# uga-ssrl/SSRLCV

Measured on AMD Instinct MI355X. Metric: Mpix/s SIFT extract (+ Mmatches/s 128-D brute-force, see `matcher`), higher is better.
Workload: dtype f32; 1 GPU; 2-view 4096x4096 pair per GPU (tools/scene.py pinhole views (PCG32 terrain + texture through Image::Camera)): SIFT_FeatureFactory::generateFeatures (sparse DoG path) on each image, pixels resident in HBM; images_per_gpu=2, parallelism=image-pair shard, library=release build (libssrlcv_hip_release.so)

## Files before the change

ssrlcv_amd/csrc/keypoints.hip:

```cpp
#include <hip/hip_runtime.h>
#include <float.h>
#include <math.h>
#include <stdlib.h>
#include "compact.h"
#include "dev_switch.h"
#include "scan_lookback.h"
#include "device_math.h"
#include "sift_plan.h"
#include "ssrlcv_hip.h"

using svp::OctaveState;

namespace {

struct LevelSet {
  const float* lvl[svp::kGauss];
  const float* lvlMinMax;
  const float* minmax;
  const float2* polar;
  int w, h;
};

struct DogView {
  const float* lo;
// ... 470 lines not shown
      tab->start[r] = pos;
      pos += count;
    }
  }
  tab->total = pos;
}
__device__ __forceinline__ int range_of(const RangeTable* tab, uint32_t u) {
  int r = 0;
#pragma unroll
  for (int k = 1; k < 20; ++k)
    if (tab->start[k] <= u) r = k;
  return r;
}

struct OctaveSet {
  LevelSet L[svp::kOctaves];
  const ssrlcv_sskeypoint* kps[svp::kOctaves];
  float pixelWidth[svp::kOctaves];
  float* thetas[svp::kOctaves];
  uint32_t* thetaCnt[svp::kOctaves];
  const void* consts[svp::kOctaves];
};

template <int MAXO, int LPKS>
__global__ __launch_bounds__(64) void k_thetas(const OctaveState* states, const RangeTable* tab, OctaveSet set, float lambda,
                                               float orientationThreshold) {
  constexpr int LANES = 1 << LPKS, PER_BLOCK = 64 >> LPKS, CW = kThetaChunk * LANES;
  __shared__ float s_hist[36][PER_BLOCK];
  if (blockIdx.x >= tab->total) return;
  const int range = __builtin_amdgcn_readfirstlane(range_of(tab, blockIdx.x));
  const int octave = range & 3, useg = kSegOrder[range >> 2];
  const LevelSet& L = set.L[octave];
  const float pixelWidth = set.pixelWidth[octave];
  const int t = threadIdx.x, sub = t & (LANES - 1), col = t >> LPKS;
  const float fsub2 = (float)(2 * sub);
  const uint32_t local = (blockIdx.x - tab->start[range]) * PER_BLOCK + (uint32_t)(t >> LPKS);
  const bool have = local < tab->count[range];
  const int gi = (int)(tab->first[range] + local);
  const float pi = SSRLCV_PI_F;
  const float rad10 = pi / 18.0f;
  const float inv10 = 1.0f / rad10;
  ssrlcv_sskeypoint kp;
  kp.loc.x = kp.loc.y = 0.0f;
  kp.sigma = 1.0f;
  if (have) kp = set.kps[octave][gi];
  const float kx = kp.loc.x, ky = kp.loc.y;
  const float windowWidth = ceilf(kp.sigma * 3.0f * lambda / pixelWidth);
  const float minx = kx - windowWidth, miny = ky - windowWidth, maxx = kx + windowWidth, maxy = ky + windowWidth;
  const bool inside = have && useg >= 1 && useg <= 3 &&
                      !(minx < 0.0f || miny < 0.0f || maxx >= (unsigned)(L.w - 1) || maxy >= (unsigned)(L.h - 1));
#pragma unroll
  for (int i = 0; i < 36 * PER_BLOCK / 64; ++i) (&s_hist[0][0])[i * 64 + t] = 0.0f;
  const float weight = 2.0f * lambda * lambda * kp.sigma * kp.sigma;
  const float rweight = 1.0f / weight;
  const int W = L.w;
  const size_t levelStride = svp::polar_level_stride(L.w, L.h);
  {
    const float2* base = L.polar + (size_t)(useg - 1) * levelStride;
    const __amdgpu_buffer_rsrc_t rsrc = __builtin_amdgcn_make_buffer_rsrc((void*)base, 0, (int)(uint32_t)(levelStride * 8), 0x00020000);
    typedef unsigned u32x4 __attribute__((ext_vector_type(4)));
    typedef unsigned u32x2 __attribute__((ext_vector_type(2)));
    struct Cursor { float x, y, ty2; unsigned rowoff; bool act; };
    Cursor cf;
    cf.x = minx;
    cf.y = miny;
    cf.ty2 = (miny - ky) * (miny - ky);
    cf.rowoff = (unsigned)round_pos(miny) * (unsigned)W + 1u;
    cf.act = inside;
    auto advance = [&](Cursor& c) {
      float xn = c.x + (float)CW;
      if (__any(c.act && !(c.x >= (float)CW))) {
        float ch = c.x;
#pragma unroll 8
        for (int i = 0; i < CW; ++i) ch += 1.0f;
        xn = c.x >= (float)CW ? xn : ch;
      }
      if (c.act) {
        if (xn <= maxx) {
          c.x = xn;
        } else {
          c.x = minx;
          c.y += 1.0f;
          if (!(c.y <= maxy)) c.act = false;
          const float ty = c.y - ky;
          c.ty2 = ty * ty;
          c.rowoff = (unsigned)round_pos(c.y) * (unsigned)W + 1u;
        }
      }
    };
    typedef u32x4 Chunk[kThetaChunk / 2];
    auto fetch = [&](const Cursor& c, Chunk& into) {
      if (!c.act) return;
      const unsigned off = (c.rowoff + (unsigned)round_pos(c.x)) * 8u + 16u * (unsigned)sub;
#pragma unroll
      for (int j = 0; j < kThetaChunk / 4; ++j) into[j] = __builtin_amdgcn_raw_buffer_load_b128(rsrc, (int)(off + 16u * LANES * j), 0, 0);
    };
    auto fetch_upper = [&](const Cursor& c, Chunk& into) {
      if (!c.act) return;
      const unsigned off = (c.rowoff + (unsigned)round_pos(c.x)) * 8u + 16u * (unsigned)sub;
#pragma unroll
      for (int j = kThetaChunk / 4; j < kThetaChunk / 2; ++j) into[j] = __builtin_amdgcn_raw_buffer_load_b128(rsrc, (int)(off + 16u * LANES * j), 0, 0);
    };
    auto wants_upper = [&](const Cursor& c) { return __any(c.act && c.x + (float)(CW / 2 - 1) <= maxx); };
    Chunk qa, qb;
    Cursor ca, cb;
#pragma unroll
    for (int j = 0; j < kThetaChunk / 2; ++j) qa[j] = qb[j] = u32x4{0u, 0u, 0u, 0u};
    ca = cf;
    fetch(cf, qa);
    if (wants_upper(cf)) fetch_upper(cf, qa);
    advance(cf);
    cb = cf;
    auto step = [&](Chunk& cur, const Cursor& cc, Chunk& nxt, Cursor& cn) __attribute__((always_inline)) {
      cn = cf;
      fetch(cf, nxt);
      if (wants_upper(cf)) fetch_upper(cf, nxt);
      advance(cf);
      float xs[kThetaChunk];
      float xlast = cc.x + (float)(CW - 1);
#pragma unroll
      for (int i = 0; i < kThetaChunk; ++i) xs[i] = cc.x + (fsub2 + (float)(((i >> 1) << (1 + LPKS)) | (i & 1)));
      if (__any(cc.act && !(cc.x >= (float)CW))) {
        float ch = cc.x;
        float xc[kThetaChunk];
#pragma unroll
        for (int sIdx = 0; sIdx < CW; ++sIdx) {
          const int q = (sIdx >> 1) & (LANES - 1), i = ((sIdx >> (1 + LPKS)) << 1) | (sIdx & 1);
          if (LANES == 1 || q == 0) xc[i] = ch;
          else xc[i] = sub == q ? ch : xc[i];
          if (sIdx + 1 < CW) ch += 1.0f;
        }
        const bool direct = cc.x >= (float)CW;
#pragma unroll
        for (int i = 0; i < kThetaChunk; ++i) xs[i] = direct ? xs[i] : xc[i];
        xlast = direct ? xlast : ch;
      }
      const float cty2 = cc.ty2;
      const unsigned crow = cc.rowoff;
      const bool cact = cc.act;
      const bool aligned = cc.x >= 4.0f && round_pos(xlast) == round_pos(cc.x) + (CW - 1);
      if (__any(cact && !aligned)) {
        if (cact && !aligned) {
#pragma unroll
          for (int i = 0; i < kThetaChunk; ++i) {
            u32x2 e = u32x2{0u, 0u};
            if (xs[i] <= maxx) e = __builtin_amdgcn_raw_buffer_load_b64(rsrc, (int)((crow + (unsigned)round_pos(xs[i])) * 8u), 0, 0);
            cur[i >> 1][(i & 1) * 2] = e[0];
            cur[i >> 1][(i & 1) * 2 + 1] = e[1];
          }
        }
      }
      auto weigh = [&](float ang, float xi, float& wgt, int& bin) {
        const float angle = fmod_2pi_above(ang + (2.0f * pi), 2.0f * pi);
        bin = (int)floorf(sv::exact_div3(angle, rad10, inv10));
        const float tx = xi - kx;
        wgt = sv::expf_nonpos(sv::exact_div5(-((tx * tx) + cty2), weight, rweight));
      };
      const bool upperHalf = __any(cact && xs[kThetaChunk / 2] <= maxx);
      float wg[kThetaChunk], mg[kThetaChunk];
      float* slot[kThetaChunk];
      auto weigh_half = [&](auto hc) __attribute__((always_inline)) {
        constexpr int i0 = decltype(hc)::value * (kThetaChunk / 2);
#pragma unroll
        for (int i = i0; i < i0 + kThetaChunk / 2; ++i) {
          const unsigned um = cur[i >> 1][(i & 1) * 2], ua = cur[i >> 1][(i & 1) * 2 + 1];
          int bin;
          weigh(__builtin_bit_cast(float, ua), xs[i], wg[i], bin);
          const bool counts = cact && xs[i] <= maxx && (unsigned)bin < 36u;
          slot[i] = &s_hist[counts ? bin : 0][col];
          mg[i] = counts ? __builtin_bit_cast(float, um) : 0.0f;
        }
      };
      auto vote_half = [&](auto hc) __attribute__((always_inline)) {
        constexpr int j0 = decltype(hc)::value * (kThetaChunk / 4);
#pragma unroll
        for (int j = j0; j < j0 + kThetaChunk / 4; ++j) {
#pragma unroll
          for (int q = 0; q < LANES; ++q) {
            if (LANES == 1 || sub == q) {
              const float h0 = *slot[2 * j], h1 = *slot[2 * j + 1];
              const float n0 = fmaf(mg[2 * j], wg[2 * j], h0);
              const float n1 = fmaf(mg[2 * j + 1], wg[2 * j + 1], slot[2 * j + 1] == slot[2 * j] ? n0 : h1);
              *slot[2 * j] = n0;
              *slot[2 * j + 1] = n1;
            }
            if (LANES > 1) __builtin_amdgcn_wave_barrier();
          }
        }
      };
      weigh_half(std::integral_constant<int, 0>{});
      if (upperHalf) weigh_half(std::integral_constant<int, 1>{});
      vote_half(std::integral_constant<int, 0>{});
      if (upperHalf) vote_half(std::integral_constant<int, 1>{});
    };
    while (__any(ca.act)) {
      step(qa, ca, qb, cb);
      if (!__any(cb.act)) break;
      step(qb, cb, qa, ca);
    }
  }
  uint32_t cnt = 0;
  float outTheta[MAXO];
#pragma unroll
  for (int i = 0; i < MAXO; ++i) outTheta[i] = -FLT_MAX;
  if (inside && sub == 0) {
    float maxHist = 0.0f;
    for (int i = 0; i < 36; ++i) {
      const float h = s_hist[i][col];
      if (h > maxHist) maxHist = h;
    }
    maxHist *= orientationThreshold;
    float bestMag[MAXO], bestTh[MAXO];
#pragma unroll
    for (int i = 0; i < MAXO; ++i) { bestMag[i] = 0.0f; bestTh[i] = 0.0f; }
    float hprev = s_hist[35][col], hb = s_hist[0][col];
    for (int b = 0; b < 36; ++b) {
      const float hnext = s_hist[b == 35 ? 0 : b + 1][col];
      if (!(hb < maxHist || hb < hprev || hb < hnext || hb < bestMag[MAXO - 1])) {
        float tmag = hb;
        float tt = (hprev - hnext) / (hprev - (2.0f * hb) + hnext);
        tt *= (pi / 36.0f);
        tt += (b * rad10);
        tt = fmodf(tt + (2.0f * pi), 2.0f * pi);
#pragma unroll
        for (int i = 0; i < MAXO; ++i) {
          if (tmag > bestMag[i]) {
#pragma unroll
            for (int ii = i; ii < MAXO; ++ii) {
              float m2 = bestMag[ii], t2 = bestTh[ii];
              bestMag[ii] = tmag;
              bestTh[ii] = tt;
              tmag = m2;
              tt = t2;
            }
          }
        }
      }
      hprev = hb;
      hb = hnext;
    }
#pragma unroll
    for (int i = 0; i < MAXO; ++i) {
      if (bestMag[i] != 0.0f) { outTheta[i] = bestTh[i]; cnt = i + 1; }
    }
  }
  if (have && sub == 0) {
#pragma unroll
    for (int i = 0; i < MAXO; ++i) set.thetas[octave][(size_t)gi * svp::kMaxOrient + i] = outTheta[i];
    set.thetaCnt[octave][gi] = cnt;
  }
}

__device__ __forceinline__ float uniform_f(float v) {
  return __builtin_bit_cast(float, __builtin_amdgcn_readfirstlane(__builtin_bit_cast(int, v)));
}
struct DescConst {
  float c, s;
  float windowWidth;
  float invExpDen;
  float voteScale;
  float invBin;
  uint32_t magic;
  int32_t segment;
};
static_assert(sizeof(DescConst) == 32, "one s_load_dwordx8");
__global__ __launch_bounds__(256) void k_desc_consts(const RangeTable* tab, OctaveSet set, float lambda, const OctaveState* states,
                                                     const GroupCtl* regularCtl) {
  const uint32_t total = tab->total;
  const bool fromTable = regularCtl != nullptr && regularCtl->regular != 0u;
  for (uint32_t u = blockIdx.x * 256 + threadIdx.x; u < total; u += gridDim.x * 256) {
    const int range = range_of(tab, u);
    const int octave = range & 3;
    const int i = (int)(tab->first[range] + (u - tab->start[range]));
    const ssrlcv_sskeypoint* kps = set.kps[octave];
    const float pixelWidth = set.pixelWidth[octave];
    DescConst* __restrict__ out = (DescConst*)const_cast<void*>(set.consts[octave]);
    DescConst d;
    const float theta = kps[i].theta;
    d.c = sv_cosf(-theta);
    d.s = sv_sinf(-theta);
    d.windowWidth = ceilf(kps[i].sigma * lambda / pixelWidth);
    d.invExpDen = 1.0f / (2.0f * d.windowWidth * d.windowWidth);
    int boundExp;
    (void)frexpf(1.4143f * ((d.windowWidth + 2.0f) * (d.windowWidth + 2.0f)), &boundExp);
    d.voteScale = ldexpf(1.0f, 31 - boundExp);
    d.invBin = 1.0f / (d.windowWidth / 2.0f);
    const unsigned wi = (unsigned)(int)d.windowWidth;
    d.magic = wi > 1u ? 0xFFFFFFFFu / wi + 1u : 0u;
    d.segment = fromTable ? kSegOrder[range >> 2] : segment_of(states + octave, i);
    out[i] = d;
  }
}

__device__ __forceinline__ unsigned vote_u32(float v) {
  int r;
  asm("v_cvt_rpi_i32_f32 %0, %1" : "=v"(r) : "v"(v));
  return (unsigned)r;
}

#ifndef SSRLCV_DESC_COPIES
#define SSRLCV_DESC_COPIES 8
#endif
constexpr int kDescCopies = SSRLCV_DESC_COPIES;
#ifndef SSRLCV_DESC_VGPRS
#define SSRLCV_DESC_VGPRS 64
#endif
__global__ __launch_bounds__(256) __attribute__((amdgpu_waves_per_eu(4, 8), amdgpu_num_vgpr(SSRLCV_DESC_VGPRS), amdgpu_num_sgpr(102))) void k_descriptors(const RangeTable* tab, OctaveSet set, const uint32_t* featBase,
                                                     ssrlcv_sift_feature* __restrict__ features, uint32_t maxFeatures) {
  __shared__ unsigned s_bins[4][(1 + 128 + 2) * kDescCopies];
  __shared__ __attribute__((aligned(8))) uint8_t s_bytes[4][128];
  const int lane = threadIdx.x & 63, wave = __builtin_amdgcn_readfirstlane(threadIdx.x >> 6);
  unsigned* bins = s_bins[wave] + kDescCopies;
  const int copy = lane & (kDescCopies - 1);
  const float pi = SSRLCV_PI_F;
  const float rad45 = pi / 4.0f;
  const float inv45 = 1.0f / rad45;
  const uint32_t totalUnits = tab->total;
  for (uint32_t unit = blockIdx.x * 4 + wave; unit < totalUnits; unit += gridDim.x * 4) {
    const int range = range_of(tab, unit);
    const int octave = range & 3;
    const int gi = (int)(tab->first[range] + (unit - tab->start[range]));
    const LevelSet& L = set.L[octave];
    const float pixelWidth = set.pixelWidth[octave];
    const float2* __restrict__ polar = L.polar;
    const DescConst dc = reinterpret_cast<const DescConst*>(set.consts[octave])[gi];
    const ssrlcv_sskeypoint kp = set.kps[octave][gi];
    const int seg = dc.segment;
    const float kx = kp.loc.x, ky = kp.loc.y;
    const float theta = kp.theta;
    const float windowWidth = dc.windowWidth;
    const float binWidth = windowWidth / 2.0f;
    const float c = dc.c, s = dc.s;
    const float2* __restrict__ pl = polar + (size_t)(seg - 1) * svp::polar_level_stride(L.w, L.h) + 1;
#pragma unroll
    for (int i = 0; i < 2 * kDescCopies; ++i) bins[i * 64 + lane] = 0u;
    f32x2 rc[16];
    {
      const int ci = lane & 15;
      const float hx = ((float)(ci >> 2) * 0.5f - 0.75f) * windowWidth, hy = ((float)(ci & 3) * 0.5f - 0.75f) * windowWidth;
      const float rx = (hx * c) + (hy * s), ry = (-hx * s) + (hy * c);
#pragma unroll
      for (int cell = 0; cell < 16; ++cell) {
        if ((cell >> 2) == 0 || (cell & 3) == 0) continue;
        rc[cell].x = __builtin_bit_cast(float, __builtin_amdgcn_readlane(__builtin_bit_cast(int, rx), cell));
        rc[cell].y = __builtin_bit_cast(float, __builtin_amdgcn_readlane(__builtin_bit_cast(int, ry), cell));
      }
    }
    const float expDen = 2.0f * windowWidth * windowWidth, invExpDen = dc.invExpDen, invBin = dc.invBin;
    const float voteScale = dc.voteScale;
    const int Wi = (int)windowWidth;
    const unsigned centreIdx = (unsigned)(Wi * (Wi + 1));
    const unsigned magic = dc.magic;
    auto sample = [&](unsigned idx, float& cx, float& cy, bool& ok) {
      const unsigned yq = Wi == 1 ? idx : __umulhi(idx, magic);
      const unsigned xq = idx - yq * (unsigned)Wi + 1u;
      const bool centre = idx >= centreIdx;
      const float x = centre ? 0.0f : (float)(int)xq;
      const float y = centre ? 0.0f : (float)(int)yq;
      cx = (x * c) + (y * s);
      cy = (-x * s) + (y * c);
      ok = idx <= centreIdx && fmaxf(fabsf(cx), fabsf(cy)) <= windowWidth;
    };
    auto gather = [&](float px, float py) { return polar_px(pl, L.w, round_coord(px), round_coord(py)); };
    auto split = [&](float2 pg, bool live, float& w0, float& w1, unsigned*& pa, float& ang, bool& odd) {
      ang = fmod_2pi_above(pg.y - theta + (2.0f * pi), 2.0f * pi);
      const float t45 = ang * inv45;
      const float fk = floorf(t45);
      const float u = t45 - fk;
      odd = live && !(u > 1.0e-4f && u < 0.9999f);
      int k0 = (int)fk;
      const float a0 = fabsf(ang - (fk * rad45)), a1 = fabsf(ang - ((fk + 1.0f) * rad45));
      w0 = (live && !odd && (unsigned)k0 < 8u) ? 1.0f - sv::exact_div3(a0, rad45, inv45) : 0.0f;
      w1 = (live && !odd && (unsigned)(k0 + 1) < 8u) ? 1.0f - sv::exact_div3(a1, rad45, inv45) : 0.0f;
      k0 = k0 < -1 ? -1 : k0;
      pa = bins + k0 * kDescCopies + copy;
    };
    float ncx, ncy;
    bool nok;
    sample((unsigned)lane, ncx, ncy, nok);
    float2 npg[4] = {make_float2(0.0f, 0.0f), make_float2(0.0f, 0.0f), make_float2(0.0f, 0.0f), make_float2(0.0f, 0.0f)};
    auto gather4 = [&]() {
      npg[0] = gather(ncx + kx, ncy + ky);
      npg[1] = gather(kx - ncy, ncx + ky);
      npg[2] = gather(kx - ncx, ky - ncy);
      npg[3] = gather(ncy + kx, ky - ncx);
    };
    if (nok) gather4();
    for (unsigned base = 0; base <= centreIdx; base += 64) {
      const float cx = ncx, cy = ncy;
      const bool ok = nok;
      const float2 pg0 = npg[0], pg1 = npg[1], pg2 = npg[2], pg3 = npg[3];
      const bool turned = ok && base + (unsigned)lane < centreIdx;
      sample(base + 64 + (unsigned)lane, ncx, ncy, nok);
      if (nok) gather4();
      const float r2n = -((cx * cx) + (cy * cy));
      const float g = sv::expf_nonpos(sv::exact_div3(r2n, expDen, invExpDen)) * voteScale;
      float a0, a1, b0, b1, c0, c1, d0, d1, angA, angB, angC, angD;
      bool oddA, oddB, oddC, oddD;
      unsigned *pa, *pb, *pc, *pd;
      split(pg0, ok, a0, a1, pa, angA, oddA);
      split(pg1, turned, b0, b1, pb, angB, oddB);
      split(pg2, turned, c0, c1, pc, angC, oddC);
      split(pg3, turned, d0, d1, pd, angD, oddD);
      const float magA = pg0.x * g, magB = pg1.x * g, magC = pg2.x * g, magD = pg3.x * g;
      const float bwl = ok ? binWidth : -1.0f;
#pragma unroll
      for (int cell = 0; cell < 16; ++cell) {
        const int nx = cell >> 2, ny = cell & 3;
        if (nx == 0 || ny == 0) continue;
        const int cellB = (3 - ny) * 4 + nx, cellC = 15 - cell, cellD = ny * 4 + (3 - nx);
        const float tx = fabsf(rc[cell].x - cx), ty = fabsf(rc[cell].y - cy);
        if (fmaxf(tx, ty) <= bwl) {
          const float wxy = (1.0f - sv::exact_div3(tx, binWidth, invBin)) * (1.0f - sv::exact_div3(ty, binWidth, invBin));
          atomicAdd(pa + cell * 8 * kDescCopies, vote_u32((wxy * a0) * magA));
          atomicAdd(pa + cell * 8 * kDescCopies + kDescCopies, vote_u32((wxy * a1) * magA));
          atomicAdd(pb + cellB * 8 * kDescCopies, vote_u32((wxy * b0) * magB));
          atomicAdd(pb + cellB * 8 * kDescCopies + kDescCopies, vote_u32((wxy * b1) * magB));
          atomicAdd(pc + cellC * 8 * kDescCopies, vote_u32((wxy * c0) * magC));
          atomicAdd(pc + cellC * 8 * kDescCopies + kDescCopies, vote_u32((wxy * c1) * magC));
          atomicAdd(pd + cellD * 8 * kDescCopies, vote_u32((wxy * d0) * magD));
          atomicAdd(pd + cellD * 8 * kDescCopies + kDescCopies, vote_u32((wxy * d1) * magD));
        }
      }
      if (__ballot(oddA || oddB || oddC || oddD) != 0ull) {
#pragma unroll 1
        for (int m = 0; m < 4; ++m) {
          const bool odd = m == 0 ? oddA : m == 1 ? oddB : m == 2 ? oddC : oddD;
          if (!odd) continue;
          const float mcx = m == 0 ? cx : m == 1 ? -cy : m == 2 ? -cx : cy;
          const float mcy = m == 0 ? cy : m == 1 ? cx : m == 2 ? -cy : -cx;
          const float mang = m == 0 ? angA : m == 1 ? angB : m == 2 ? angC : angD;
          const float mmag = m == 0 ? magA : m == 1 ? magB : m == 2 ? magC : magD;
#pragma unroll 1
          for (int cell = 0; cell < 16; ++cell) {
            const int ci = lane & 15;
            (void)ci;
            const float hx0 = ((float)(cell >> 2) * 0.5f - 0.75f) * windowWidth, hy0 = ((float)(cell & 3) * 0.5f - 0.75f) * windowWidth;
            const float rx = (hx0 * c) + (hy0 * s), ry = (-hx0 * s) + (hy0 * c);
            float hx = fabsf(rx - mcx), hy = fabsf(ry - mcy);
            if (hx <= binWidth && hy <= binWidth) {
              hx = hx / binWidth;
              hy = hy / binWidth;
              for (int k = 0; k < 8; ++k) {
                float angle = fabsf(mang - ((float)k * rad45));
                if (angle < rad45) {
                  angle /= rad45;
                  const float temp = (1.0f - hx) * (1.0f - hy) * (1.0f - angle) * mmag;
                  atomicAdd(bins + (cell * 8 + k) * kDescCopies + copy, vote_u32(temp));
                }
              }
            }
          }
        }
      }
    }
    __builtin_amdgcn_wave_barrier();
    unsigned t0 = 0u, t1 = 0u;
#pragma unroll
    for (int cpy = 0; cpy < kDescCopies; ++cpy) {
      t0 += bins[lane * kDescCopies + cpy];
      t1 += bins[(lane + 64) * kDescCopies + cpy];
    }
    float v0 = (float)t0, v1 = (float)t1;
    float sq = sqrtf(sv::wave_sum((v0 * v0) + (v1 * v1)));
    v0 = v0 / sq;
    v1 = v1 / sq;
    if (v0 > 0.2f) v0 = 0.2f;
    if (v1 > 0.2f) v1 = 0.2f;
    sq = sqrtf(sv::wave_sum((v0 * v0) + (v1 * v1)));
    {
      int b0 = lane, b1 = lane + 64;
      int o0 = (((b0 >> 3) & 3) * 4 + (b0 >> 5)) * 8 + (b0 & 7);
      int o1 = (((b1 >> 3) & 3) * 4 + (b1 >> 5)) * 8 + (b1 & 7);
      s_bytes[wave][o0] = (uint8_t)roundf(255.0f * v0 / sq);
      s_bytes[wave][o1] = (uint8_t)roundf(255.0f * v1 / sq);
    }
    __builtin_amdgcn_wave_barrier();
    const uint32_t fi = featBase[octave] + (uint32_t)gi;
    if (fi < maxFeatures) {
      ssrlcv_sift_feature* f = features + fi;
      if (lane < 16) *reinterpret_cast<uint2*>(&f->values[lane * 8]) = *reinterpret_cast<const uint2*>(&s_bytes[wave][lane * 8]);
      if (lane == 16) {
        f->parent = -1;
        reinterpret_cast<int*>(f)[1] = 0;
        f->theta = kp.theta;
        f->sigma = kp.sigma;
        f->loc.x = kp.loc.x * pixelWidth;
        f->loc.y = kp.loc.y * pixelWidth;
      }
    }
    __builtin_amdgcn_wave_barrier();
  }
}

LevelSet make_levels(const ssrlcv_sift_plan* plan, char* ws, int o) {
  LevelSet L;
  const svp::OctavePlan& oc = plan->oct[o];
  for (int b = 0; b < svp::kGauss; ++b) L.lvl[b] = (const float*)(ws + plan->off_gauss[o][b]);
  L.lvlMinMax = (const float*)(ws + plan->off_minmax) + (size_t)o * 2 * (svp::kGauss + svp::kDog);
  L.minmax = L.lvlMinMax + 2 * svp::kGauss;
  L.polar = (const float2*)(ws + oc.off_polar);
  L.w = (int)oc.w;
  L.h = (int)oc.h;
  return L;
}

void launch_polar(const ssrlcv_sift_plan* plan, char* ws, hipStream_t st, int oFirst = 0, int oLast = svp::kOctaves - 1) {
  PolarJobs jobs;
  uint32_t pos = 0;
  for (int o = 0; o < svp::kOctaves; ++o) {
    const svp::OctavePlan& oc = plan->oct[o];
    jobs.L[o] = make_levels(plan, ws, o);
    jobs.out[o] = (float2*)(ws + oc.off_polar);
    jobs.start[o] = pos;
    jobs.tilesX[o] = (oc.w + 255) / 256;
    if (o >= oFirst && o <= oLast) pos += jobs.tilesX[o] * ((oc.h + kPolRows - 1) / kPolRows);
  }
  jobs.start[svp::kOctaves] = pos;
  hipLaunchKernelGGL(k_polar, dim3(pos), dim3(256), 0, st, jobs);
}

}
namespace svp {
void launch_polar_octave(const ssrlcv_sift_plan* plan, char* ws, int octave, hipStream_t st) {
  PolarJobs jobs;
  const svp::OctavePlan& oc = plan->oct[octave];
  const uint32_t tilesX = (oc.w + 255) / 256, tiles = tilesX * ((oc.h + kPolRows - 1) / kPolRows);
  for (int o = 0; o < svp::kOctaves; ++o) {
    jobs.L[o] = make_levels(plan, ws, octave);
    jobs.out[o] = (float2*)(ws + oc.off_polar);
    jobs.tilesX[o] = tilesX;
    jobs.start[o] = o <= octave ? 0u : tiles;
  }
  jobs.start[svp::kOctaves] = tiles;
  hipLaunchKernelGGL(k_polar, dim3(tiles), dim3(256), 0, st, jobs);
}
}
namespace {
hipError_t run_discard(OctaveState* st, const ssrlcv_sskeypoint* src, ssrlcv_sskeypoint* dst, uint32_t cap,
                       uint32_t* words, hipStream_t stream) {
  const OctaveState* cst = st;
  auto keyfn = [=] __device__(uint32_t i) -> uint32_t {
    if (!cst->hasExtrema || (int)i >= cst->n) return 0u;
    if (src[i].discard) return 0u;
    return 1u << segment_of(cst, (int)i);
  };
  auto emit = [=] __device__(uint32_t i, int, uint32_t d) { dst[d] = src[i]; };
  uint32_t* totals = nullptr;
  auto post = [=] __device__(const uint32_t* tot) { book_discard(st, tot); };
  return svc::partition<svp::kDog, 8>(cap, keyfn, emit, words, &totals, stream, &st->n, 1u, post);
}

constexpr unsigned kWaveKernelOversubscription = 16;
inline unsigned list_blocks(uint32_t cap) {
  unsigned b = (cap + 255) / 256;
  return b > 1024 ? 1024 : b;
}

}

extern "C" {

int ssrlcv_sift_plan_keypoints(const ssrlcv_sift_plan* plan, void* workspace, int octave, ssrlcv_sskeypoint** list,
                               int** blurIndices_dev) {
  if (!plan || !workspace || octave < 0 || octave >= svp::kOctaves) return SSRLCV_ERR_INVALID_ARG;
  char* ws = (char*)workspace;
  if (list) *list = (ssrlcv_sskeypoint*)(ws + (plan->listInB[octave] ? plan->oct[octave].off_kpB : plan->oct[octave].off_kpA));
  if (blurIndices_dev) *blurIndices_dev = (int*)(ws + plan->off_state + sizeof(OctaveState) * octave);
  return SSRLCV_OK;
}

int ssrlcv_sift_plan_overflow(const ssrlcv_sift_plan* plan, const void* workspace, uint32_t* octaveMask,
                              ssrlcv_stream_t stream) {
  if (!plan || !workspace || !octaveMask) return SSRLCV_ERR_INVALID_ARG;
  OctaveState st[svp::kOctaves];
  SSRLCV_HIP_TRY(hipMemcpyAsync(st, (const char*)workspace + plan->off_state, sizeof st, hipMemcpyDeviceToHost,
                                (hipStream_t)stream));
  SSRLCV_HIP_TRY(hipStreamSynchronize((hipStream_t)stream));
  uint32_t m = 0;
  for (int o = 0; o < svp::kOctaves; ++o)
    if (st[o].overflow) m |= 1u << o;
  *octaveMask = m;
  return m ? SSRLCV_ERR_CAPACITY : SSRLCV_OK;
}

}
namespace {

struct ListCtx {
  const ssrlcv_sift_plan* plan;
  const svp::OctavePlan* oc;
  int o;
  hipStream_t s;
  OctaveState* st;
  LevelSet L;
  ssrlcv_sskeypoint *A, *B;
  uint8_t* flags;
  uint32_t* words;
  uint32_t cap;
  ssrlcv_sskeypoint* cur() const { return plan->listInB[o] ? B : A; }
  ssrlcv_sskeypoint* oth() const { return plan->listInB[o] ? A : B; }
  void flip() const { plan->listInB[o] ^= 1; }
};
ListCtx make_ctx(const ssrlcv_sift_plan* plan, char* ws, int o, hipStream_t s) {
  ListCtx c;
  c.plan = plan;
  c.oc = &plan->oct[o];
  c.o = o;
  c.s = s;
  c.st = (OctaveState*)(ws + plan->off_state) + o;
  c.L = make_levels(plan, ws, o);
  c.A = (ssrlcv_sskeypoint*)(ws + c.oc->off_kpA);
  c.B = (ssrlcv_sskeypoint*)(ws + c.oc->off_kpB);
  c.flags = (uint8_t*)(ws + c.oc->off_flags);
  c.words = (uint32_t*)(ws + c.oc->off_part);
  c.cap = c.oc->cap;
  return c;
}

int stage_extrema(const ListCtx& c, bool afterFirstNoise) {
  hipLaunchKernelGGL(k_state_reset, dim3(1), dim3(1), 0, c.s, c.st);
  c.plan->listInB[c.o] = 0;
  const uint32_t P = c.oc->w * c.oc->h, cap = c.cap;
  const int W = (int)c.oc->w;
  const int octaveId = c.o;
  const float s1 = c.oc->sigma[1], s2 = c.oc->sigma[2], s3 = c.oc->sigma[3];
  const LevelSet Lc = c.L;
  ssrlcv_sskeypoint* first = c.A;
  auto emit = [=] __device__(uint32_t p, int b, uint32_t d) {
    if (d >= cap) return;
    ssrlcv_sskeypoint kp;
    kp.octave = octaveId;
    kp.blur = (int)b + 1;
    kp.loc.x = (float)(p % W);
    kp.loc.y = (float)(p / W);
    kp.intensity = dog_view(Lc, b + 1).raw(p);
    kp.sigma = b == 0 ? s1 : b == 1 ? s2 : s3;
    kp.theta = -1.0f;
    kp.discard = 0;
    first[d] = kp;
  };
  uint32_t* totals = nullptr;
  hipError_t e = svc::partition_flags<3>(P, c.flags, afterFirstNoise ? svp::kNoiseFlagShift : 0, emit, c.words, &totals, c.s);
  if (e != hipSuccess) return (int)e;
  hipLaunchKernelGGL(k_book_extrema, dim3(1), dim3(1), 0, c.s, c.st, totals, cap);
  return SSRLCV_OK;
}
int discard_flagged(const ListCtx& c) {
  hipError_t e = run_discard(c.st, c.cur(), c.oth(), c.cap, c.words, c.s);
  if (e != hipSuccess) return (int)e;
  c.flip();
  return SSRLCV_OK;
}
int stage_noise(const ListCtx& c, float threshold) {
  hipLaunchKernelGGL(k_flag_noise, dim3(list_blocks(c.cap)), dim3(256), 0, c.s, c.st, c.cur(), threshold);
  return discard_flagged(c);
}
int stage_refine(const ListCtx& c) {
  hipLaunchKernelGGL(k_refine, dim3(list_blocks(c.cap)), dim3(256), 0, c.s, c.st, c.cur(), c.L, c.oc->sigma[0],
                     c.oc->sigma[1] / c.oc->sigma[0]);
  int rc = discard_flagged(c);
  if (rc) return rc;
  OctaveState* st = c.st;
  const OctaveState* cst = c.st;
  const ssrlcv_sskeypoint* src = c.cur();
  ssrlcv_sskeypoint* dst = c.oth();
  auto keyfn = [=] __device__(uint32_t i) -> uint32_t {
    if (!cst->hasExtrema || (int)i >= cst->n) return 0u;
    int b = src[i].blur;
    return (b < 0 || b >= svp::kDog) ? 0u : (1u << b);
  };
  auto emit = [=] __device__(uint32_t i, int, uint32_t d) { dst[d] = src[i]; };
  uint32_t* totals = nullptr;
  auto post = [=] __device__(const uint32_t* tot) { book_rescan(st, tot); };
  hipError_t e = svc::partition<svp::kDog, 8>(c.cap, keyfn, emit, c.words, &totals, c.s, &st->n, 1u, post);
  if (e != hipSuccess) return (int)e;
  c.flip();
  return SSRLCV_OK;
}
int stage_edges(const ListCtx& c) {
  hipLaunchKernelGGL(k_flag_edges, dim3(list_blocks(c.cap)), dim3(256), 0, c.s, c.st, c.cur(), c.L, svp::kEdgeThreshold);
  return discard_flagged(c);
}
int stage_window(const ListCtx& c) {
  hipLaunchKernelGGL(k_flag_window, dim3(list_blocks(c.cap)), dim3(256), 0, c.s, c.st, c.cur(), c.L.w, c.L.h, c.oc->pixelWidth,
                     c.plan->params.descriptorContribWidth);
  return discard_flagged(c);
}
int stage_noise_edges_window(const ListCtx& c) {
  hipLaunchKernelGGL(k_flag_noise_edges_window, dim3(list_blocks(c.cap)), dim3(256), 0, c.s, c.st, c.cur(), c.L, svp::kNoiseThreshold,
                     svp::kEdgeThreshold, c.oc->pixelWidth, c.plan->params.descriptorContribWidth);
  return discard_flagged(c);
}

OctaveSet make_set(const ssrlcv_sift_plan* plan, char* ws) {
// ... 993 lines not shown
```

Before: 3595 Mpix/s.

## Add packed in-window sample enumeration and interior-keypoint fast gather to descriptor kernel

Adds an optional packed sampling mode that builds, per keypoint, a row table of the in-window x range in LDS and enumerates only valid samples, so lanes are not spent on points rejected by the rotated-window test. The mode is off by default through a macro. It also adds an interior-keypoint path that uses a cheaper rounding (round_pos) when the window cannot go negative, and it forces bin pointers into the LDS address space so the compiler emits ds ops. The default path gains the inner branch and the address-space cast, and the loop bound now uses `last`, which equals centreIdx when packing is off.

```diff
diff --git a/ssrlcv_amd/csrc/keypoints.hip b/ssrlcv_amd/csrc/keypoints.hip
--- a/ssrlcv_amd/csrc/keypoints.hip
+++ b/ssrlcv_amd/csrc/keypoints.hip
@@ -796,6 +796,10 @@
 #define SSRLCV_DESC_COPIES 8
 #endif
 constexpr int kDescCopies = SSRLCV_DESC_COPIES;
+#ifndef SSRLCV_DESC_PACKED
+#define SSRLCV_DESC_PACKED 0
+#endif
+typedef __attribute__((address_space(3))) unsigned lds_u32;
 #ifndef SSRLCV_DESC_VGPRS
 #define SSRLCV_DESC_VGPRS 64
 #endif
@@ -826,6 +830,43 @@
     const float binWidth = windowWidth / 2.0f;
     const float c = dc.c, s = dc.s;
     const float2* __restrict__ pl = polar + (size_t)(seg - 1) * svp::polar_level_stride(L.w, L.h) + 1;
+    const int Wi = (int)windowWidth;
+    const unsigned centreIdx = (unsigned)(Wi * (Wi + 1));
+    unsigned last = centreIdx;
+    unsigned start16 = 0u;
+    const uint32_t* rowTab = reinterpret_cast<const uint32_t*>(s_bytes[wave]);
+    const bool packed = SSRLCV_DESC_PACKED != 0 && Wi <= 31;
+    if (packed) {
+      int ln = lane;
+      asm volatile("" : "+v"(ln));
+      const int row = ln & 31, half = (Wi + 1) >> 1, x0 = ln < 32 ? 1 : half + 1;
+      const float y = (float)row;
+      const float ys = y * s, yc = y * c;
+      unsigned lo = 0u, hi = 0u;
+#pragma unroll 1
+      for (int i = 0; i < half; ++i) {
+        const int xi = x0 + i;
+        const float x = (float)xi;
+        const float cx = (x * c) + ys, cy = (-x * s) + yc;
+        if (xi <= Wi && row <= Wi && fmaxf(fabsf(cx), fabsf(cy)) <= windowWidth) {
+          lo = lo == 0u ? (unsigned)xi : lo;
+          hi = (unsigned)xi;
+        }
+      }
+      const unsigned upper = (unsigned)__builtin_amdgcn_ds_bpermute((ln ^ 32) << 2, (int)(lo | hi << 8));
+      const unsigned rowLo = lo != 0u ? lo : upper & 0xFFu, rowHi = upper != 0u ? upper >> 8 : hi;
+      const unsigned rowN = ln < 32 && rowLo != 0u ? rowHi - rowLo + 1u : 0u;
+      unsigned incl = rowN;
+#pragma unroll
+      for (int o = 1; o < 32; o <<= 1) {
+        const unsigned below = (unsigned)__builtin_amdgcn_ds_bpermute((ln - o) << 2, (int)incl);
+        if (ln >= o) incl += below;
+      }
+      const unsigned word = (incl - rowN) | rowLo << 16;
+      if (ln < 32) reinterpret_cast<uint32_t*>(s_bytes[wave])[ln] = word;
+      start16 = (unsigned)__builtin_amdgcn_readlane((int)word, 16) & 0xFFFFu;
+      last = (unsigned)__builtin_amdgcn_readlane((int)incl, 31);
+    }
 #pragma unroll
     for (int i = 0; i < 2 * kDescCopies; ++i) bins[i * 64 + lane] = 0u;
     f32x2 rc[16];
@@ -842,20 +883,30 @@
     }
     const float expDen = 2.0f * windowWidth * windowWidth, invExpDen = dc.invExpDen, invBin = dc.invBin;
     const float voteScale = dc.voteScale;
-    const int Wi = (int)windowWidth;
-    const unsigned centreIdx = (unsigned)(Wi * (Wi + 1));
     const unsigned magic = dc.magic;
     auto sample = [&](unsigned idx, float& cx, float& cy, bool& ok) {
-      const unsigned yq = Wi == 1 ? idx : __umulhi(idx, magic);
-      const unsigned xq = idx - yq * (unsigned)Wi + 1u;
-      const bool centre = idx >= centreIdx;
+      unsigned xq, yq;
+      if (packed) {
+        yq = start16 <= idx ? 16u : 0u;
+#pragma unroll
+        for (unsigned step = 8u; step != 0u; step >>= 1)
+          if ((rowTab[yq + step] & 0xFFFFu) <= idx) yq += step;
+        const unsigned e = rowTab[yq];
+        xq = (e >> 16) + (idx - (e & 0xFFFFu));
+      } else {
+        yq = Wi == 1 ? idx : __umulhi(idx, magic);
+        xq = idx - yq * (unsigned)Wi + 1u;
+      }
+      const bool centre = idx >= last;
       const float x = centre ? 0.0f : (float)(int)xq;
       const float y = centre ? 0.0f : (float)(int)yq;
       cx = (x * c) + (y * s);
       cy = (-x * s) + (y * c);
-      ok = idx <= centreIdx && fmaxf(fabsf(cx), fabsf(cy)) <= windowWidth;
+      ok = idx <= last && fmaxf(fabsf(cx), fabsf(cy)) <= windowWidth;
     };
+    const bool inner = kx - windowWidth > -0.5f && ky - windowWidth > -0.5f;
     auto gather = [&](float px, float py) { return polar_px(pl, L.w, round_coord(px), round_coord(py)); };
+    auto gather_inner = [&](float px, float py) { return polar_px(pl, L.w, round_pos(px), round_pos(py)); };
     auto split = [&](float2 pg, bool live, float& w0, float& w1, unsigned*& pa, float& ang, bool& odd) {
       ang = fmod_2pi_above(pg.y - theta + (2.0f * pi), 2.0f * pi);
       const float t45 = ang * inv45;
@@ -868,23 +919,33 @@
       w1 = (live && !odd && (unsigned)(k0 + 1) < 8u) ? 1.0f - sv::exact_div3(a1, rad45, inv45) : 0.0f;
       k0 = k0 < -1 ? -1 : k0;
       pa = bins + k0 * kDescCopies + copy;
+      unsigned addr = (unsigned)(uintptr_t)(lds_u32*)pa;
+      asm("" : "+v"(addr));
+      pa = (unsigned*)(lds_u32*)(uintptr_t)addr;
     };
     float ncx, ncy;
     bool nok;
     sample((unsigned)lane, ncx, ncy, nok);
     float2 npg[4] = {make_float2(0.0f, 0.0f), make_float2(0.0f, 0.0f), make_float2(0.0f, 0.0f), make_float2(0.0f, 0.0f)};
     auto gather4 = [&]() {
-      npg[0] = gather(ncx + kx, ncy + ky);
-      npg[1] = gather(kx - ncy, ncx + ky);
-      npg[2] = gather(kx - ncx, ky - ncy);
-      npg[3] = gather(ncy + kx, ky - ncx);
+      if (inner) {
+        npg[0] = gather_inner(ncx + kx, ncy + ky);
+        npg[1] = gather_inner(kx - ncy, ncx + ky);
+        npg[2] = gather_inner(kx - ncx, ky - ncy);
+        npg[3] = gather_inner(ncy + kx, ky - ncx);
+      } else {
+        npg[0] = gather(ncx + kx, ncy + ky);
+        npg[1] = gather(kx - ncy, ncx + ky);
+        npg[2] = gather(kx - ncx, ky - ncy);
+        npg[3] = gather(ncy + kx, ky - ncx);
+      }
     };
     if (nok) gather4();
-    for (unsigned base = 0; base <= centreIdx; base += 64) {
+    for (unsigned base = 0; base <= last; base += 64) {
       const float cx = ncx, cy = ncy;
       const bool ok = nok;
       const float2 pg0 = npg[0], pg1 = npg[1], pg2 = npg[2], pg3 = npg[3];
-      const bool turned = ok && base + (unsigned)lane < centreIdx;
+      const bool turned = ok && base + (unsigned)lane < last;
       sample(base + 64 + (unsigned)lane, ncx, ncy, nok);
       if (nok) gather4();
       const float r2n = -((cx * cx) + (cy * cy));
```

Measured after the change: 3597 Mpix/s (median of 4 runs). No clear change (+0.1%).
